# ndas7/Parallel-Systems-MPI-TFIDF

Hardware: AMD Instinct MI355X
Metric: corpus GB/s (TF-IDF hot path: tokenize->TF->DF->tf*idf->ordered output) (higher is better)
Workload: dtype u8/u32 (f64 score)

## Files before the change

parallel-systems-mpi-tfidf_amd/csrc/finalize.hip:

```cpp
#include "dev_common.h"
#include "dev_vocab.h"
#include "kernels.h"
#include "synth.h"

#include <type_traits>
#define G(p) ((GLOBAL_AS std::remove_pointer_t<decltype(p)>*)(p))
template <class T> __device__ __forceinline__ void sto(T* p, T v) { *(GLOBAL_AS T*)p = v; }

namespace {
constexpr int NT = 256;
inline unsigned grid_for(uint64_t n, int nt = NT) { return n ? (unsigned)((n + nt - 1) / nt) : 1u; }
inline int ok() { return hipGetLastError() == hipSuccess ? 0 : -1; }

__device__ __forceinline__ uint4 u128_from(uint64_t lo, uint64_t hi) {
    return make_uint4((uint32_t)lo, (uint32_t)(lo >> 32), (uint32_t)hi, (uint32_t)(hi >> 32));
}
__device__ __forceinline__ bool u128_eq(uint4 a, uint4 b) { return a.x == b.x && a.y == b.y && a.z == b.z && a.w == b.w; }
}


__global__ void k_vocab_flags(VocabDev v, uint64_t cap, uint32_t* __restrict__ flags) {
    uint64_t s = (uint64_t)blockIdx.x * blockDim.x + threadIdx.x;
    if (s >= cap) return;
    uint4 k = v.keys[s];
// ... 971 lines not shown
    k_df_mark<<<grid_for(V), NT, 0, s>>>(df, V, present);
    return ok();
}
__global__ void k_df_list(const uint32_t* __restrict__ ps, uint64_t nvals, uint32_t* __restrict__ vals) {
    const uint64_t stride = (uint64_t)gridDim.x * blockDim.x;
    for (uint64_t x = (uint64_t)blockIdx.x * blockDim.x + threadIdx.x; x < nvals; x += stride)
        if (ps[x + 1] != ps[x]) vals[ps[x]] = (uint32_t)x;
}
int launch_df_list(const uint32_t* present_scan, uint64_t nvals, uint32_t* vals, hipStream_t s) {
    const unsigned full = grid_for(nvals), cap = 1u << 20;
    k_df_list<<<full < cap ? full : cap, NT, 0, s>>>(present_scan, nvals, vals);
    return ok();
}


__global__ void k_doc_keys(const uint32_t* __restrict__ ids, uint32_t n, uint64_t* __restrict__ keys,
                           uint32_t* __restrict__ seq) {
    uint32_t i = blockIdx.x * blockDim.x + threadIdx.x;
    if (i >= n) return;
    uint32_t id = ids ? ids[i] : i + 1;
    uint32_t dg[10];
    int k = 0;
    do { dg[k++] = id % 10; id /= 10; } while (id);
    uint64_t key = 0;
    for (int p = 0; p < 10; ++p) key = key * 11 + (p < k ? dg[k - 1 - p] : 10u);
    keys[i] = key;
    seq[i] = i;
}
int launch_doc_keys(const uint32_t* doc_ids, uint32_t ndocs, uint64_t* keys, uint32_t* seq, hipStream_t s) {
    if (!ndocs) return 0;
    k_doc_keys<<<grid_for(ndocs), NT, 0, s>>>(doc_ids, ndocs, keys, seq);
    return ok();
}
__global__ void k_gather_meta(const uint32_t* __restrict__ order, const uint32_t* __restrict__ np,
                              const uint64_t* __restrict__ recoff, const uint32_t* __restrict__ dsize,
                              const uint8_t* __restrict__ flags, uint32_t n, uint64_t* __restrict__ out,
                              uint4* __restrict__ meta) {
    uint32_t i = blockIdx.x * blockDim.x + threadIdx.x;
    if (i >= n) return;
    const uint32_t d = order[i];
    const uint32_t c = np[d];
    const uint64_t rb = c ? recoff[d] : 0ull;
    out[i] = c;
    meta[i] = make_uint4((uint32_t)rb, (uint32_t)(rb >> 32), (c & 0x3FFFFFFFu) | ((uint32_t)(flags[d] & 3u) << 30), dsize[d]);
}
int launch_gather_meta(const uint32_t* order, const uint32_t* doc_npairs, const uint64_t* doc_recoff,
                       const uint32_t* doc_size, const uint8_t* doc_flags, uint32_t ndocs, uint64_t* npairs_ord,
                       uint4* meta, hipStream_t s) {
    if (!ndocs) return 0;
    k_gather_meta<<<grid_for(ndocs), NT, 0, s>>>(order, doc_npairs, doc_recoff, doc_size, doc_flags, ndocs,
                                                npairs_ord, meta);
    return ok();
}


constexpr int K5_MAX = K5_MAX_PAIRS;
constexpr uint32_t K5_SMALL = 64;
constexpr uint32_t K5_SMALL_DOC = 128;
constexpr uint32_t K5_PS_SPLIT = 4096;
constexpr uint32_t K5_WAVE = 1024;
constexpr uint32_t K5_IDX_BITS = 11;
constexpr int K5_BATCH = 8;
#ifndef K5_EB
#define K5_EB 4
#endif
#ifndef K5_EMIT
#define K5_EMIT 2
#endif
#ifndef K5_WPS
#define K5_WPS 4
#endif
#ifndef K5_WPS_WIDE
#define K5_WPS_WIDE 4
#endif
constexpr uint32_t K5_NB_BITS = 9;
constexpr uint32_t K5_NB = 1u << K5_NB_BITS;
constexpr uint32_t K5_GROUP_MAX = 48;
constexpr uint32_t K5L_GROUP_MAX = 32;
#ifndef K5L_EB
#define K5L_EB 8
#endif

__global__ void k_idf_of_rank(const uint32_t* __restrict__ df_of_rank, const uint32_t* __restrict__ idf_idx,
                              const double* __restrict__ idf, uint32_t V, double* __restrict__ out) {
    uint32_t r = blockIdx.x * blockDim.x + threadIdx.x;
    if (r < V) out[r] = idf_idx ? idf[idf_idx[df_of_rank[r]]] : idf[df_of_rank[r]];
}

template <bool BYDF>
__device__ __forceinline__ double k5_idf(const K5Args& a, uint32_t r) {
    if constexpr (BYDF) return G(a.idf)[G(a.df_of_rank)[r]];
    else return G(a.idf_rank)[r];
}

template <bool BYDF>
__device__ __forceinline__ void k5_emit(const K5Args& a, uint64_t o, double ds, uint32_t rank, uint32_t cnt) {
    const double tf = (double)cnt / ds;
    sto(&a.out_term[o], (uint32_t)(rank));
    sto(&a.out_cnt[o], (uint32_t)(cnt));
    sto(&a.out_score[o], (double)(tf * k5_idf<BYDF>(a, rank)));
}

__device__ __forceinline__ uint32_t k5_rank(const K5Args& a, uint32_t r) {
    if (r >= a.nterms) { atomicOr(a.status, ST_BOUNDS); r = 0; }
    return r;
}

constexpr uint32_t K5_WIDE_BITS = 32 - K5_IDX_BITS + K5_NB_BITS;
__device__ __forceinline__ bool k5_by_wave(const K5Args& a, uint32_t n, bool presorted) {
    if (presorted) return n <= K5_WAVE;
    return n <= K5_SMALL || (n <= K5_WAVE && a.rank_bits <= K5_WIDE_BITS);
}

__device__ __noinline__ void k5_radix(uint32_t rank_bits, const uint32_t* rec_cnt, const double* idf_rank,
                                      uint32_t* out_term, uint32_t* out_cnt, double* out_score, uint32_t* buf0,
                                      uint32_t* buf1, uint32_t* h, uint32_t n, uint64_t rb, uint64_t ob, double ds) {
    const uint32_t lane = threadIdx.x & 63;
    const uint64_t below = (1ull << lane) - 1ull;
    uint32_t cur = 0;
    for (uint32_t sh = K5_IDX_BITS; sh < K5_IDX_BITS + rank_bits; sh += 8) {
        const uint32_t* src = cur ? buf1 : buf0;
        uint32_t* dst = cur ? buf0 : buf1;
        h[4 * lane] = 0; h[4 * lane + 1] = 0; h[4 * lane + 2] = 0; h[4 * lane + 3] = 0;
        __builtin_amdgcn_fence(__ATOMIC_RELEASE, "wavefront");
        __builtin_amdgcn_fence(__ATOMIC_ACQUIRE, "wavefront");
        for (uint32_t j = lane; j < n; j += 64) atomicAdd(&h[(src[j] >> sh) & 0xFFu], 1u);
        __builtin_amdgcn_fence(__ATOMIC_RELEASE, "wavefront");
        __builtin_amdgcn_fence(__ATOMIC_ACQUIRE, "wavefront");
        {
            const uint32_t v0 = h[4 * lane], v1 = h[4 * lane + 1], v2 = h[4 * lane + 2], v3 = h[4 * lane + 3];
            const uint32_t tot = v0 + v1 + v2 + v3;
            const uint32_t ex = wave_incl_scan(tot) - tot;
            h[4 * lane] = ex; h[4 * lane + 1] = ex + v0; h[4 * lane + 2] = ex + v0 + v1; h[4 * lane + 3] = ex + v0 + v1 + v2;
        }
        __builtin_amdgcn_fence(__ATOMIC_RELEASE, "wavefront");
        __builtin_amdgcn_fence(__ATOMIC_ACQUIRE, "wavefront");
        for (uint32_t r0 = 0; r0 < n; r0 += 64) {
            const uint32_t j = r0 + lane;
            const bool valid = j < n;
            const uint32_t key = valid ? src[j] : 0u;
            const uint32_t dg = (key >> sh) & 0xFFu;
            uint64_t m = __ballot(valid);
#pragma unroll
            for (int b = 0; b < 8; ++b) {
                const bool bit = (dg >> b) & 1u;
                const uint64_t bb = __ballot(valid && bit);
                m &= bit ? bb : ~bb;
            }
            const uint32_t lrank = (uint32_t)__popcll(m & below);
            const uint32_t cnt = (uint32_t)__popcll(m);
            const uint32_t base = valid ? h[dg] : 0u;
            __builtin_amdgcn_fence(__ATOMIC_RELEASE, "wavefront");
            __builtin_amdgcn_fence(__ATOMIC_ACQUIRE, "wavefront");
            if (valid) {
                dst[base + lrank] = key;
                if (lrank == cnt - 1u) h[dg] = base + cnt;
            }
            __builtin_amdgcn_fence(__ATOMIC_RELEASE, "wavefront");
            __builtin_amdgcn_fence(__ATOMIC_ACQUIRE, "wavefront");
        }
        cur ^= 1u;
    }
    const uint32_t* fin = cur ? buf1 : buf0;
    for (uint32_t j0 = 0; j0 < n; j0 += 64 * K5_BATCH) {
        uint32_t key[K5_BATCH], cnt[K5_BATCH];
        double idf[K5_BATCH];
#pragma unroll
        for (int q = 0; q < K5_BATCH; ++q) {
// ... 698 lines not shown
            }
            __builtin_amdgcn_fence(__ATOMIC_RELEASE, "wavefront");
            __builtin_amdgcn_fence(__ATOMIC_ACQUIRE, "wavefront");
        }
#pragma unroll
        for (int q = 0; q < Q; ++q) {
            if (64u * q + lane < n) {
                const uint64_t o = D0.ob + pos[q];
                sto(&a.out_term[o], (uint32_t)(r0[q]));
                sto(&a.out_cnt[o], (uint32_t)(c0[q]));
                sto(&a.out_score[o], (double)(((double)c0[q] / D0.ds) * f0[q]));
            }
        }
        D0 = D1;
        D1 = D2;
#pragma unroll
        for (int q = 0; q < Q; ++q) {
            r0[q] = r1[q]; c0[q] = c1[q]; f0[q] = f1[q];
            r1[q] = r2[q]; c1[q] = c2[q];
        }
    }
}
template <bool BYDF>
__global__ __launch_bounds__(256) void k_emit_split(K5Args a) {
    const uint32_t nt = *a.split_count < a.split_cap ? *a.split_count : a.split_cap;
    for (uint32_t t = blockIdx.x; t < nt; t += gridDim.x) {
        const uint2 tk = a.split_tasks[t];
        const uint4 m = gload(a.meta + tk.x);
        const uint32_t n = m.z & 0x3FFFFFFFu;
        const uint64_t rb = ((uint64_t)m.y << 32) | m.x;
        const uint64_t ob = G(a.out_off)[tk.x];
        const double ds = (double)m.w;
        if (rb + n > a.rec_total) { if (threadIdx.x == 0) atomicOr(a.status, ST_BOUNDS); continue; }
        const uint32_t j1 = (tk.y + 1) * K5_PS_SPLIT < n ? (tk.y + 1) * K5_PS_SPLIT : n;
        for (uint32_t j0 = tk.y * K5_PS_SPLIT; j0 < j1; j0 += 256 * K5L_EB) {
            uint32_t rk[K5L_EB], cn[K5L_EB];
            double f[K5L_EB];
#pragma unroll
            for (int e = 0; e < K5L_EB; ++e) {
                const uint32_t j = j0 + 256u * e + threadIdx.x;
                rk[e] = j < j1 ? a.rec_slot[rb + j] : 0u;
                cn[e] = j < j1 ? a.rec_cnt[rb + j] : 0u;
            }
#pragma unroll
            for (int e = 0; e < K5L_EB; ++e) {
                const uint32_t j = j0 + 256u * e + threadIdx.x;
                if (j < j1) rk[e] = k5_rank(a, rk[e]);
                f[e] = j < j1 ? k5_idf<BYDF>(a, rk[e]) : 0.0;
            }
#pragma unroll
            for (int e = 0; e < K5L_EB; ++e) {
                const uint32_t j = j0 + 256u * e + threadIdx.x;
                if (j < j1) {
                    sto(&a.out_term[ob + j], (uint32_t)(rk[e]));
                    sto(&a.out_cnt[ob + j], (uint32_t)(cn[e]));
                    sto(&a.out_score[ob + j], (double)(((double)cn[e] / ds) * f[e]));
                }
            }
        }
    }
}
static void launch_score_wave(const K5Args& a, bool wide, uint32_t wg, hipStream_t s) {
    if (!wide) k_score_wave<false, false><<<wg, NT, 0, s>>>(a);
    else if (a.idf_by_df) k_score_wave<true, true><<<wg, NT, 0, s>>>(a);
    else k_score_wave<true, false><<<wg, NT, 0, s>>>(a);
}
static void launch_emit_split(const K5Args& a, int ncu, hipStream_t s) {
    if (a.idf_by_df) k_emit_split<true><<<(unsigned)ncu * 4u, 256, 0, s>>>(a);
    else k_emit_split<false><<<(unsigned)ncu * 4u, 256, 0, s>>>(a);
}
static void launch_score_large(const K5Args& a, uint32_t grid, hipStream_t s) {
    static_assert(K5_MAX % 2 == 0 && K5_MAX / 2 >= 1024, "k_score_large instances");
    if (a.idf_by_df) {
        k_score_large<(uint32_t)K5_MAX / 2, 10, true><<<grid, NT, 0, s>>>(a);
        k_score_large<(uint32_t)K5_MAX, 11, true><<<grid, NT, 0, s>>>(a);
    } else {
        k_score_large<(uint32_t)K5_MAX / 2, 10, false><<<grid, NT, 0, s>>>(a);
        k_score_large<(uint32_t)K5_MAX, 11, false><<<grid, NT, 0, s>>>(a);
    }
}
int launch_score_order(const K5Args& a, Arena& ar, hipStream_t s, hipStream_t s2, hipEvent_t ev_fork,
                       hipEvent_t ev_join) {
    if (!a.ndocs) return 0;
    {
        FillList fl{};
        fl.p[0] = a.large_count;
        fl.bytes[0] = 4;
        fl.n = 1;
        if (a.split_count) {
            fl.p[1] = a.split_count;
            fl.bytes[1] = 4;
            fl.n = 2;
        }
        if (launch_fill_multi(fl, s)) return -1;
    }
    if (!a.idf_by_df)
        k_idf_of_rank<<<grid_for(a.nterms ? a.nterms : 1), NT, 0, s>>>(a.df_of_rank, a.idf_idx, a.idf, a.nterms,
                                                                      a.idf_rank);
    static int ncu = 0;
    if (!ncu) {
        int dev = 0;
        if (hipGetDevice(&dev) != hipSuccess ||
            hipDeviceGetAttribute(&ncu, hipDeviceAttributeMultiprocessorCount, dev) != hipSuccess || ncu <= 0)
            ncu = 256;
    }
    const uint32_t wg_need = (a.ndocs + NT / 64 - 1) / (NT / 64);
    const bool wide = a.rank_bits + K5_IDX_BITS > 32;
    const uint32_t wg_cu = wide ? (uint32_t)K5_WPS_WIDE : 4u;
    const uint32_t wg = wg_need < (uint32_t)ncu * wg_cu ? wg_need : (uint32_t)ncu * wg_cu;
    const uint32_t grid = a.ndocs < 2048u ? a.ndocs : 2048u;
    K5Args hand = a;
    hand.cls_list = nullptr;
    if (!a.cls_list || !a.cls_off) return -1;
    k_k5_classify<<<a.cls_nblk, 256, 0, s>>>(a);
    if (scan_excl_u32(a.cls_off, a.cls_off, 3ull * a.cls_nblk + 1, ar, s)) return -1;
    k_k5_scatter<<<a.cls_nblk, 256, 0, s>>>(a);
    if (a.idf_by_df && !wide) return -1;
    if (a.idf_by_df) k_score_small<true><<<(unsigned)ncu * (unsigned)K5S_OCC, 256, 0, s>>>(a);
    else k_score_small<false><<<(unsigned)ncu * (unsigned)K5S_OCC, 256, 0, s>>>(a);
    launch_score_wave(a, wide, wg, s);
    if (a.split_count) launch_emit_split(a, ncu, s);
    launch_score_large(a, grid, s);
    if (wide) launch_score_large(hand, grid, s);
    return ok();
}


__global__ void k_keys_by_rank(const uint4* __restrict__ vkeys, const uint32_t* __restrict__ slot_of_rank, uint32_t V,
                               uint4* __restrict__ out) {
    uint32_t r = blockIdx.x * blockDim.x + threadIdx.x;
    if (r < V) out[r] = vkeys[slot_of_rank[r]];
}
int launch_keys_by_rank(const uint4* vkeys, const uint32_t* slot_of_rank, uint32_t V, uint4* out, hipStream_t s) {
    if (!V) return 0;
    k_keys_by_rank<<<grid_for(V), NT, 0, s>>>(vkeys, slot_of_rank, V, out);
    return ok();
}
__device__ __forceinline__ uint32_t owner_of(const uint4 k, uint32_t R) {
    const uint64_t lo = ((uint64_t)k.y << 32) | k.x, hi = ((uint64_t)k.w << 32) | k.z;
    const uint64_t h = mix64(lo ^ (hi * 0x9E3779B97F4A7C15ull) ^ 0x5851F42D4C957F2Dull);
    return (uint32_t)(((h >> 32) * (uint64_t)R) >> 32);
}
constexpr uint32_t XO_MAXR = 1024;
__device__ __forceinline__ uint4 owner_key(const OwnerKeySrc& ks, uint32_t i) {
    const uint4 s = gload(ks.skey + i);
    const uint32_t b15 = s.x & 0xFFu;
    if (b15 == 0x00u || b15 == 0x09u)
        return make_uint4(__builtin_bswap32(s.w), __builtin_bswap32(s.z), __builtin_bswap32(s.y), __builtin_bswap32(s.x));
    return gload(ks.vkeys + G(ks.slot_of_rank)[i]);
}
__global__ void k_owner_count(const OwnerKeySrc ks, uint32_t V, uint32_t R, uint32_t* __restrict__ cnt) {
    __shared__ uint32_t h[XO_MAXR];
    for (uint32_t o = threadIdx.x; o < R; o += blockDim.x) h[o] = 0;
    __syncthreads();
    for (uint32_t r = blockIdx.x * blockDim.x + threadIdx.x; r < V; r += gridDim.x * blockDim.x)
        atomicAdd(&h[owner_of(owner_key(ks, r), R)], 1u);
    __syncthreads();
    for (uint32_t o = threadIdx.x; o < R; o += blockDim.x)
        if (h[o]) atomicAdd(&cnt[o], h[o]);
}
__global__ void k_owner_scatter(const OwnerKeySrc ks, const uint32_t* __restrict__ df, uint32_t V, uint32_t R,
                                const uint32_t* __restrict__ cnt, uint32_t* __restrict__ cur, uint32_t* __restrict__ srec,
                                uint32_t* __restrict__ sidx) {
    __shared__ uint32_t h[XO_MAXR], base[XO_MAXR], seg[XO_MAXR];
    if (threadIdx.x == 0) {
        uint32_t acc = 0;
        for (uint32_t o = 0; o < R; ++o) { seg[o] = acc; acc += cnt[o]; }
    }
    for (uint32_t o = threadIdx.x; o < R; o += blockDim.x) h[o] = 0;
    __syncthreads();
    const uint32_t r0 = blockIdx.x * blockDim.x * 8;
    uint32_t own[8], pos[8];
#pragma unroll
    for (int q = 0; q < 8; ++q) {
        const uint32_t r = r0 + q * blockDim.x + threadIdx.x;
        own[q] = r < V ? owner_of(owner_key(ks, r), R) : 0xFFFFFFFFu;
        pos[q] = own[q] != 0xFFFFFFFFu ? atomicAdd(&h[own[q]], 1u) : 0u;
    }
    __syncthreads();
    for (uint32_t o = threadIdx.x; o < R; o += blockDim.x) base[o] = h[o] ? seg[o] + atomicAdd(&cur[o], h[o]) : 0u;
    __syncthreads();
// ... 695 lines not shown
```

parallel-systems-mpi-tfidf_amd/csrc/prims.hip:

```cpp
#include "prims.h"
#include "dev_common.h"

namespace {

constexpr int SC_NT = 256;
constexpr int SC_IT = 8;
constexpr int SC_TILE = SC_NT * SC_IT;

template <typename T>
__device__ __forceinline__ T wave_incl_scan_t(T v) {
    const int lane = threadIdx.x & 63;
#pragma unroll
    for (int o = 1; o < 64; o <<= 1) {
        T t = __shfl_up(v, o, 64);
        if (lane >= o) v += t;
    }
    return v;
}

template <typename T>
__device__ __forceinline__ T block_excl_scan_t(T v, T* wsum, T* total) {
    const int lane = threadIdx.x & 63, w = threadIdx.x >> 6;
    T inc = wave_incl_scan_t(v);
    if (lane == 63) wsum[w] = inc;
// ... 167 lines not shown
    for (int j = 0; j < RS_IT; ++j) {
        const uint64_t idx = wb + (uint64_t)j * 64 + lane;
        const bool valid = idx < n;
        k[j] = valid ? kin[idx] : K{};
        v[j] = valid ? vin[idx] : 0u;
        d[j] = valid ? digit_of(k[j], p) : 0u;
    }
#pragma unroll
    for (int j = 0; j < RS_IT; ++j) {
        const bool valid = wb + (uint64_t)j * 64 + lane < n;
        uint64_t m = __ballot(valid);
#pragma unroll
        for (int b = 0; b < 8; ++b) {
            const bool bit = (d[j] >> b) & 1u;
            const uint64_t bb = __ballot(valid && bit);
            m &= bit ? bb : ~bb;
        }
        const uint32_t lrank = (uint32_t)__popcll(m & lt);
        r[j] = valid ? wc[w][d[j]] + lrank : 0u;
        if (valid && lrank == 0) wc[w][d[j]] += (uint32_t)__popcll(m);
    }
    __syncthreads();
    {
        uint32_t c[RS_NT / 64], tot = 0;
#pragma unroll
        for (int q = 0; q < RS_NT / 64; ++q) { c[q] = wc[q][tid]; wc[q][tid] = tot; tot += c[q]; }
        uint32_t all;
        dstart[tid] = block_excl_scan<RS_NT>(tot, wsum, &all);
    }
    __syncthreads();
#pragma unroll
    for (int j = 0; j < RS_IT; ++j) {
        if (wb + (uint64_t)j * 64 + lane >= n) continue;
        const uint32_t pos = dstart[d[j]] + wc[w][d[j]] + r[j];
        sk[pos] = k[j];
        sv[pos] = v[j];
    }
    __syncthreads();
    const uint32_t tn = n - t0 < (uint64_t)RS_TILE ? (uint32_t)(n - t0) : (uint32_t)RS_TILE;
#pragma unroll
    for (int q = 0; q < RS_IT; ++q) {
        const uint32_t i = (uint32_t)tid + (uint32_t)q * RS_NT;
        if (i >= tn) continue;
        const K kk = sk[i];
        const uint32_t dd = digit_of(kk, p);
        const uint64_t o = (uint64_t)gbase[dd] + (i - dstart[dd]);
        kout[o] = kk;
        vout[o] = sv[i];
    }
}

template <typename K>
int radix_sort_t(K* k0, uint32_t* v0, K* k1, uint32_t* v1, uint64_t n, uint32_t byte_mask, int nbytes,
                 Arena& ar, hipStream_t s) {
    if (n <= 1 || byte_mask == 0) return 0;
    if (n > 0xFFFFFFFFull) return -3;
    uint32_t nb = (uint32_t)((n + RS_TILE - 1) / RS_TILE);
    size_t m = ar.mark();
    uint32_t* hist = (uint32_t*)ar.get(((uint64_t)256 * nb + 1) * sizeof(uint32_t));
    if (!hist) return -2;
    int cur = 0;
    for (int p = 0; p < nbytes; ++p) {
        if (!((byte_mask >> p) & 1u)) continue;
        K* ki = cur ? k1 : k0;
        uint32_t* vi = cur ? v1 : v0;
        K* ko = cur ? k0 : k1;
        uint32_t* vo = cur ? v0 : v1;
        k_rs_hist<K><<<nb, RS_NT, 0, s>>>(ki, n, p, hist, nb);
        if (nb <= RS_FUSED_MAXNB) {
            k_rs_scatter<K, true><<<nb, RS_NT, 0, s>>>(ki, vi, ko, vo, n, p, hist, nb);
        } else {
            int rc = scan_excl_t<uint32_t>(hist, hist, (uint64_t)256 * nb, ar, s);
            if (rc) return rc;
            k_rs_scatter<K, false><<<nb, RS_NT, 0, s>>>(ki, vi, ko, vo, n, p, hist, nb);
        }
        cur ^= 1;
    }
    ar.release(m);
    return hipGetLastError() == hipSuccess ? cur : -1;
}

constexpr int TS_NT = 1024;
constexpr uint32_t TS_T = 2048;

__device__ __forceinline__ bool key_lt(uint64_t a, uint64_t b) { return a < b; }
__device__ __forceinline__ bool key_eq(uint64_t a, uint64_t b) { return a == b; }
__device__ __forceinline__ bool key_lt(uint4 a, uint4 b) {
    if (a.w != b.w) return a.w < b.w;
    if (a.z != b.z) return a.z < b.z;
    if (a.y != b.y) return a.y < b.y;
    return a.x < b.x;
}
__device__ __forceinline__ bool key_eq(uint4 a, uint4 b) { return a.x == b.x && a.y == b.y && a.z == b.z && a.w == b.w; }
__device__ __forceinline__ void key_max(uint64_t& k) { k = ~0ull; }
__device__ __forceinline__ void key_max(uint4& k) { k = make_uint4(~0u, ~0u, ~0u, ~0u); }

template <typename K>
__global__ __launch_bounds__(TS_NT) void k_tile_sort(const K* __restrict__ kin, const uint32_t* __restrict__ vin,
                                                    uint64_t n, K* __restrict__ tk, uint32_t* __restrict__ tv,
                                                    uint32_t* __restrict__ ti) {
    __shared__ K sk[TS_T];
    __shared__ uint32_t sv[TS_T], si[TS_T];
    const uint32_t tid = threadIdx.x;
    const uint64_t t0 = (uint64_t)blockIdx.x * TS_T;
#pragma unroll
    for (uint32_t h = 0; h < 2; ++h) {
        const uint32_t e = tid + h * TS_NT;
        const uint64_t g = t0 + e;
        if (g < n) { sk[e] = kin[g]; sv[e] = vin[g]; si[e] = (uint32_t)g; }
        else { K m; key_max(m); sk[e] = m; sv[e] = 0u; si[e] = 0xFFFFFFFFu; }
    }
    __syncthreads();
    for (uint32_t k = 2; k <= TS_T; k <<= 1) {
        for (uint32_t j = k >> 1; j > 0; j >>= 1) {
            const uint32_t i = 2u * tid - (tid & (j - 1u)), l = i + j;
            const bool asc = (i & k) == 0u;
            const K a = sk[i], b = sk[l];
            const uint32_t ia = si[i], ib = si[l];
            const bool b_first = key_lt(b, a) || (key_eq(a, b) && ib < ia);
            if (b_first == asc) {
                sk[i] = b; sk[l] = a;
                si[i] = ib; si[l] = ia;
                const uint32_t x = sv[i]; sv[i] = sv[l]; sv[l] = x;
            }
            __syncthreads();
        }
    }
#pragma unroll
    for (uint32_t h = 0; h < 2; ++h) {
        const uint32_t e = tid + h * TS_NT;
        const uint64_t g = t0 + e;
        if (g < n) { tk[g] = sk[e]; tv[g] = sv[e]; ti[g] = si[e]; }
    }
}

constexpr uint32_t TS_LB = 8;
template <typename K>
__global__ __launch_bounds__(256) void k_tile_rank(const K* __restrict__ tk, const uint32_t* __restrict__ ti,
                                                  uint64_t n, uint32_t* __restrict__ pos) {
    const uint64_t g = (uint64_t)blockIdx.x * blockDim.x + threadIdx.x;
    if (g >= n) return;
    const uint32_t t = (uint32_t)(g / TS_T), nt = (uint32_t)((n + TS_T - 1) / TS_T);
    const uint32_t b0 = blockIdx.y * TS_LB;
    const K key = tk[g];
    const uint32_t idx = ti[g];
    uint32_t lo[TS_LB], len[TS_LB];
#pragma unroll
    for (uint32_t q = 0; q < TS_LB; ++q) {
        const uint32_t b = b0 + q;
        const uint64_t st = (uint64_t)b * TS_T;
        lo[q] = 0;
        len[q] = (b < nt && b != t) ? (uint32_t)((n - st) < TS_T ? (n - st) : TS_T) : 0u;
    }
    for (uint32_t it = 0; it < 12; ++it) {
#pragma unroll
        for (uint32_t q = 0; q < TS_LB; ++q) {
            if (len[q] == 0u) continue;
            const uint32_t half = len[q] >> 1, mid = lo[q] + half;
            const uint64_t e = (uint64_t)(b0 + q) * TS_T + mid;
            const K m = tk[e];
            const bool before = key_lt(m, key) || (key_eq(m, key) && ti[e] < idx);
            if (before) { lo[q] = mid + 1u; len[q] -= half + 1u; }
            else len[q] = half;
        }
    }
    uint32_t c = blockIdx.y == 0 ? (uint32_t)(g - (uint64_t)t * TS_T) : 0u;
#pragma unroll
    for (uint32_t q = 0; q < TS_LB; ++q) c += lo[q];
    if (c) atomicAdd(&pos[g], c);
}
template <typename K>
__global__ void k_tile_place(const K* __restrict__ tk, const uint32_t* __restrict__ tv,
                             const uint32_t* __restrict__ pos, uint64_t n, K* __restrict__ kout,
                             uint32_t* __restrict__ vout) {
    const uint64_t g = (uint64_t)blockIdx.x * blockDim.x + threadIdx.x;
    if (g >= n) return;
    const uint32_t p = pos[g];
    kout[p] = tk[g];
    vout[p] = tv[g];
}

template <typename K>
int tile_sort_t(const K* k0, const uint32_t* v0, K* k1, uint32_t* v1, uint64_t n, Arena& ar, hipStream_t s) {
    if (n == 0) return 1;
    const uint32_t nt = (uint32_t)((n + TS_T - 1) / TS_T);
    size_t m = ar.mark();
    K* tk = (K*)ar.get(n * sizeof(K));
    uint32_t* tv = (uint32_t*)ar.get(n * 4);
    uint32_t* ti = (uint32_t*)ar.get(n * 4);
    if (!tk || !tv || !ti) return -2;
    uint32_t* pos = (uint32_t*)ar.get(n * 4);
    if (!pos) return -2;
    if (hipMemsetAsync(pos, 0, n * 4, s) != hipSuccess) return -1;
    k_tile_sort<K><<<nt, TS_NT, 0, s>>>(k0, v0, n, tk, tv, ti);
    k_tile_rank<K><<<dim3((unsigned)((n + 255) / 256), (nt + TS_LB - 1) / TS_LB), 256, 0, s>>>(tk, ti, n, pos);
    k_tile_place<K><<<(unsigned)((n + 255) / 256), 256, 0, s>>>(tk, tv, pos, n, k1, v1);
    ar.release(m);
    return hipGetLastError() == hipSuccess ? 1 : -1;
}

__global__ __launch_bounds__(256) void k_orand_u64(const uint64_t* __restrict__ k, uint64_t n, unsigned long long* acc) {
    __shared__ unsigned long long sa[4], so[4];
    uint64_t a = ~0ull, o = 0;
    for (uint64_t i = (uint64_t)blockIdx.x * blockDim.x + threadIdx.x; i < n; i += (uint64_t)gridDim.x * blockDim.x) {
        a &= k[i];
        o |= k[i];
    }
    for (int off = 32; off > 0; off >>= 1) {
        a &= __shfl_xor(a, off, 64);
        o |= __shfl_xor(o, off, 64);
    }
    const int w = threadIdx.x >> 6;
    if ((threadIdx.x & 63) == 0) { sa[w] = a; so[w] = o; }
    __syncthreads();
    if (threadIdx.x == 0) {
        atomicAnd(&acc[0], sa[0] & sa[1] & sa[2] & sa[3]);
        atomicOr(&acc[1], so[0] | so[1] | so[2] | so[3]);
    }
}

__global__ __launch_bounds__(256) void k_orand_u128(const uint4* __restrict__ k, uint64_t n, unsigned long long* acc) {
    __shared__ unsigned long long s4[4][4];
    uint64_t a0 = ~0ull, a1 = ~0ull, o0 = 0, o1 = 0;
    for (uint64_t i = (uint64_t)blockIdx.x * blockDim.x + threadIdx.x; i < n; i += (uint64_t)gridDim.x * blockDim.x) {
        uint4 v = k[i];
        uint64_t lo = ((uint64_t)v.y << 32) | v.x, hi = ((uint64_t)v.w << 32) | v.z;
        a0 &= lo; a1 &= hi; o0 |= lo; o1 |= hi;
    }
    for (int off = 32; off > 0; off >>= 1) {
        a0 &= __shfl_xor(a0, off, 64); a1 &= __shfl_xor(a1, off, 64);
        o0 |= __shfl_xor(o0, off, 64); o1 |= __shfl_xor(o1, off, 64);
    }
    const int w = threadIdx.x >> 6;
    if ((threadIdx.x & 63) == 0) { s4[w][0] = a0; s4[w][1] = a1; s4[w][2] = o0; s4[w][3] = o1; }
    __syncthreads();
    if (threadIdx.x == 0) {
        atomicAnd(&acc[0], s4[0][0] & s4[1][0] & s4[2][0] & s4[3][0]);
        atomicAnd(&acc[1], s4[0][1] & s4[1][1] & s4[2][1] & s4[3][1]);
        atomicOr(&acc[2], s4[0][2] | s4[1][2] | s4[2][2] | s4[3][2]);
        atomicOr(&acc[3], s4[0][3] | s4[1][3] | s4[2][3] | s4[3][3]);
    }
}

}

int scan_excl_u32(const uint32_t* in, uint32_t* out, uint64_t n, Arena& ar, hipStream_t s) {
    return scan_excl_t<uint32_t>(in, out, n, ar, s);
}
int scan_excl_u64(const uint64_t* in, uint64_t* out, uint64_t n, Arena& ar, hipStream_t s) {
    return scan_excl_t<uint64_t>(in, out, n, ar, s);
}
int tile_sort_u64(const uint64_t* k0, const uint32_t* v0, uint64_t* k1, uint32_t* v1, uint64_t n, Arena& ar,
                  hipStream_t s) {
    if (n > SORT_TILE_MAXN) return -3;
    if (n <= 1) {
        if (n == 1 && (hipMemcpyAsync(k1, k0, 8, hipMemcpyDeviceToDevice, s) != hipSuccess ||
                       hipMemcpyAsync(v1, v0, 4, hipMemcpyDeviceToDevice, s) != hipSuccess)) return -1;
        return 1;
    }
    return tile_sort_t<uint64_t>(k0, v0, k1, v1, n, ar, s);
}
int tile_sort_u128(const uint4* k0, const uint32_t* v0, uint4* k1, uint32_t* v1, uint64_t n, Arena& ar,
                   hipStream_t s) {
    if (n > SORT_TILE_MAXN) return -3;
    if (n <= 1) {
        if (n == 1 && (hipMemcpyAsync(k1, k0, 16, hipMemcpyDeviceToDevice, s) != hipSuccess ||
                       hipMemcpyAsync(v1, v0, 4, hipMemcpyDeviceToDevice, s) != hipSuccess)) return -1;
        return 1;
    }
    return tile_sort_t<uint4>(k0, v0, k1, v1, n, ar, s);
}
int radix_sort_u64(uint64_t* k0, uint32_t* v0, uint64_t* k1, uint32_t* v1, uint64_t n, uint32_t byte_mask,
                   Arena& ar, hipStream_t s) {
    return radix_sort_t<uint64_t>(k0, v0, k1, v1, n, byte_mask, 8, ar, s);
}
int radix_sort_u128(uint4* k0, uint32_t* v0, uint4* k1, uint32_t* v1, uint64_t n, uint32_t byte_mask,
                    Arena& ar, hipStream_t s) {
    return radix_sort_t<uint4>(k0, v0, k1, v1, n, byte_mask, 16, ar, s);
}
// ... 75 lines not shown
```

Before: 337.2.

## Fuse tile-sort rank and place into block-level merge-path kernel, drop value shuffling

Replaces the per-element global binary-search ranking kernel plus separate placement kernel with one kernel. In it, each 256-key block finds its window in every other tile using wave-cooperative 64-way search, then ranks window elements against the block's keys held in LDS, and scatters directly. The tile sort stops carrying values through the bitonic network, gathers them by original index instead, and uses wavefront barriers for small strides. A single-tile fast path skips the rank pass entirely. Separately, zeroing of the counters is folded into the idf kernel to save a fill launch. The cost is a much more intricate kernel with LDS sizing tied to SORT_TILE_MAXN, plus a fallback path for wide windows.

```diff
diff --git a/parallel-systems-mpi-tfidf_amd/csrc/finalize.hip b/parallel-systems-mpi-tfidf_amd/csrc/finalize.hip
--- a/parallel-systems-mpi-tfidf_amd/csrc/finalize.hip
+++ b/parallel-systems-mpi-tfidf_amd/csrc/finalize.hip
@@ -1077,8 +1077,13 @@
 #endif
 
 __global__ void k_idf_of_rank(const uint32_t* __restrict__ df_of_rank, const uint32_t* __restrict__ idf_idx,
-                              const double* __restrict__ idf, uint32_t V, double* __restrict__ out) {
+                              const double* __restrict__ idf, uint32_t V, double* __restrict__ out,
+                              uint32_t* __restrict__ z0, uint32_t* __restrict__ z1) {
     uint32_t r = blockIdx.x * blockDim.x + threadIdx.x;
+    if (r == 0) {
+        *z0 = 0u;
+        if (z1) *z1 = 0u;
+    }
     if (r < V) out[r] = idf_idx ? idf[idf_idx[df_of_rank[r]]] : idf[df_of_rank[r]];
 }
 
@@ -1943,7 +1948,10 @@
 int launch_score_order(const K5Args& a, Arena& ar, hipStream_t s, hipStream_t s2, hipEvent_t ev_fork,
                        hipEvent_t ev_join) {
     if (!a.ndocs) return 0;
-    {
+    if (!a.idf_by_df) {
+        k_idf_of_rank<<<grid_for(a.nterms ? a.nterms : 1), NT, 0, s>>>(a.df_of_rank, a.idf_idx, a.idf, a.nterms,
+                                                                      a.idf_rank, a.large_count, a.split_count);
+    } else {
         FillList fl{};
         fl.p[0] = a.large_count;
         fl.bytes[0] = 4;
@@ -1955,9 +1963,6 @@
         }
         if (launch_fill_multi(fl, s)) return -1;
     }
-    if (!a.idf_by_df)
-        k_idf_of_rank<<<grid_for(a.nterms ? a.nterms : 1), NT, 0, s>>>(a.df_of_rank, a.idf_idx, a.idf, a.nterms,
-                                                                      a.idf_rank);
     static int ncu = 0;
     if (!ncu) {
         int dev = 0;
diff --git a/parallel-systems-mpi-tfidf_amd/csrc/prims.hip b/parallel-systems-mpi-tfidf_amd/csrc/prims.hip
--- a/parallel-systems-mpi-tfidf_amd/csrc/prims.hip
+++ b/parallel-systems-mpi-tfidf_amd/csrc/prims.hip
@@ -273,119 +273,265 @@
 
 constexpr int TS_NT = 1024;
 constexpr uint32_t TS_T = 2048;
-
-__device__ __forceinline__ bool key_lt(uint64_t a, uint64_t b) { return a < b; }
-__device__ __forceinline__ bool key_eq(uint64_t a, uint64_t b) { return a == b; }
-__device__ __forceinline__ bool key_lt(uint4 a, uint4 b) {
-    if (a.w != b.w) return a.w < b.w;
-    if (a.z != b.z) return a.z < b.z;
-    if (a.y != b.y) return a.y < b.y;
-    return a.x < b.x;
-}
-__device__ __forceinline__ bool key_eq(uint4 a, uint4 b) { return a.x == b.x && a.y == b.y && a.z == b.z && a.w == b.w; }
+constexpr uint32_t TS_WSPAN = 128;
+
 __device__ __forceinline__ void key_max(uint64_t& k) { k = ~0ull; }
 __device__ __forceinline__ void key_max(uint4& k) { k = make_uint4(~0u, ~0u, ~0u, ~0u); }
+__device__ __forceinline__ uint64_t key_hi(uint64_t k) { return k; }
+__device__ __forceinline__ uint64_t key_hi(uint4 k) { return ((uint64_t)k.w << 32) | k.z; }
+__device__ __forceinline__ bool pair_before(uint64_t a, uint32_t ia, uint64_t b, uint32_t ib) {
+    return (a < b) | ((a == b) & (ia < ib));
+}
+__device__ __forceinline__ bool pair_before(uint4 a, uint32_t ia, uint4 b, uint32_t ib) {
+    const uint64_t ah = ((uint64_t)a.w << 32) | a.z, al = ((uint64_t)a.y << 32) | a.x;
+    const uint64_t bh = ((uint64_t)b.w << 32) | b.z, bl = ((uint64_t)b.y << 32) | b.x;
+    return (ah < bh) | ((ah == bh) & ((al < bl) | ((al == bl) & (ia < ib))));
+}
 
 template <typename K>
 __global__ __launch_bounds__(TS_NT) void k_tile_sort(const K* __restrict__ kin, const uint32_t* __restrict__ vin,
-                                                    uint64_t n, K* __restrict__ tk, uint32_t* __restrict__ tv,
-                                                    uint32_t* __restrict__ ti) {
+                                                    uint64_t n, uint32_t tl, K* __restrict__ tk,
+                                                    uint32_t* __restrict__ ti, uint32_t* __restrict__ vout) {
     __shared__ K sk[TS_T];
-    __shared__ uint32_t sv[TS_T], si[TS_T];
+    __shared__ uint32_t si[TS_T];
     const uint32_t tid = threadIdx.x;
-    const uint64_t t0 = (uint64_t)blockIdx.x * TS_T;
+    const uint64_t t0 = (uint64_t)blockIdx.x * tl;
 #pragma unroll
     for (uint32_t h = 0; h < 2; ++h) {
         const uint32_t e = tid + h * TS_NT;
         const uint64_t g = t0 + e;
-        if (g < n) { sk[e] = kin[g]; sv[e] = vin[g]; si[e] = (uint32_t)g; }
-        else { K m; key_max(m); sk[e] = m; sv[e] = 0u; si[e] = 0xFFFFFFFFu; }
-    }
-    __syncthreads();
+        if (e < tl && g < n) { sk[e] = kin[g]; si[e] = (uint32_t)g; }
+        else { K m; key_max(m); sk[e] = m; si[e] = 0xFFFFFFFFu; }
+    }
+    lds_barrier();
     for (uint32_t k = 2; k <= TS_T; k <<= 1) {
         for (uint32_t j = k >> 1; j > 0; j >>= 1) {
             const uint32_t i = 2u * tid - (tid & (j - 1u)), l = i + j;
             const bool asc = (i & k) == 0u;
             const K a = sk[i], b = sk[l];
             const uint32_t ia = si[i], ib = si[l];
-            const bool b_first = key_lt(b, a) || (key_eq(a, b) && ib < ia);
-            if (b_first == asc) {
+            if (pair_before(b, ib, a, ia) == asc) {
                 sk[i] = b; sk[l] = a;
                 si[i] = ib; si[l] = ia;
-                const uint32_t x = sv[i]; sv[i] = sv[l]; sv[l] = x;
-            }
-            __syncthreads();
+            }
+            const uint32_t nj = j > 1u ? j >> 1 : k;
+            if (j >= TS_WSPAN || nj >= TS_WSPAN) lds_barrier();
+            else {
+                __builtin_amdgcn_fence(__ATOMIC_RELEASE, "wavefront");
+                __builtin_amdgcn_wave_barrier();
+                __builtin_amdgcn_fence(__ATOMIC_ACQUIRE, "wavefront");
+            }
         }
     }
 #pragma unroll
     for (uint32_t h = 0; h < 2; ++h) {
         const uint32_t e = tid + h * TS_NT;
         const uint64_t g = t0 + e;
-        if (g < n) { tk[g] = sk[e]; tv[g] = sv[e]; ti[g] = si[e]; }
-    }
-}
-
-constexpr uint32_t TS_LB = 8;
+        if (e >= tl || g >= n) continue;
+        const uint32_t src = si[e];
+        tk[g] = sk[e];
+        if (vout) vout[g] = src < n ? vin[src] : 0u;
+        else ti[g] = src;
+    }
+}
+
+constexpr int TR_NT = 1024;
+constexpr uint32_t TR_K = 256;
+constexpr uint32_t TR_U = 8;
+constexpr uint32_t TR_SR = 2u * 64u / (TR_NT / 64u);
+constexpr uint32_t TR_WMAX = 512;
+constexpr uint32_t TR_FL = 4;
+constexpr uint32_t TR_MAXT = (uint32_t)(SORT_TILE_MAXN / TS_T);
 template <typename K>
-__global__ __launch_bounds__(256) void k_tile_rank(const K* __restrict__ tk, const uint32_t* __restrict__ ti,
-                                                  uint64_t n, uint32_t* __restrict__ pos) {
-    const uint64_t g = (uint64_t)blockIdx.x * blockDim.x + threadIdx.x;
-    if (g >= n) return;
-    const uint32_t t = (uint32_t)(g / TS_T), nt = (uint32_t)((n + TS_T - 1) / TS_T);
-    const uint32_t b0 = blockIdx.y * TS_LB;
-    const K key = tk[g];
-    const uint32_t idx = ti[g];
-    uint32_t lo[TS_LB], len[TS_LB];
-#pragma unroll
-    for (uint32_t q = 0; q < TS_LB; ++q) {
-        const uint32_t b = b0 + q;
-        const uint64_t st = (uint64_t)b * TS_T;
-        lo[q] = 0;
-        len[q] = (b < nt && b != t) ? (uint32_t)((n - st) < TS_T ? (n - st) : TS_T) : 0u;
-    }
-    for (uint32_t it = 0; it < 12; ++it) {
-#pragma unroll
-        for (uint32_t q = 0; q < TS_LB; ++q) {
-            if (len[q] == 0u) continue;
-            const uint32_t half = len[q] >> 1, mid = lo[q] + half;
-            const uint64_t e = (uint64_t)(b0 + q) * TS_T + mid;
-            const K m = tk[e];
-            const bool before = key_lt(m, key) || (key_eq(m, key) && ti[e] < idx);
-            if (before) { lo[q] = mid + 1u; len[q] -= half + 1u; }
-            else len[q] = half;
-        }
-    }
-    uint32_t c = blockIdx.y == 0 ? (uint32_t)(g - (uint64_t)t * TS_T) : 0u;
-#pragma unroll
-    for (uint32_t q = 0; q < TS_LB; ++q) c += lo[q];
-    if (c) atomicAdd(&pos[g], c);
-}
-template <typename K>
-__global__ void k_tile_place(const K* __restrict__ tk, const uint32_t* __restrict__ tv,
-                             const uint32_t* __restrict__ pos, uint64_t n, K* __restrict__ kout,
-                             uint32_t* __restrict__ vout) {
-    const uint64_t g = (uint64_t)blockIdx.x * blockDim.x + threadIdx.x;
-    if (g >= n) return;
-    const uint32_t p = pos[g];
-    kout[p] = tk[g];
-    vout[p] = tv[g];
+__global__ __launch_bounds__(TR_NT) void k_tile_rank_place(const K* __restrict__ tk, const uint32_t* __restrict__ ti,
+                                                          const uint32_t* __restrict__ vin, uint64_t n, uint32_t tl,
+                                                          K* __restrict__ kout, uint32_t* __restrict__ vout) {
+    __shared__ K bk[TR_K];
+    __shared__ uint64_t bh[TR_K];
+    __shared__ uint32_t bi[TR_K];
+    __shared__ uint32_t wlo[TR_MAXT], whi[TR_MAXT], woff[TR_MAXT + 1], big[TR_MAXT];
+    __shared__ uint32_t hist[TR_K + 1], fwd[TR_K];
+    __shared__ uint32_t wsum[TR_NT / 64];
+    __shared__ uint32_t sbase, nbig;
+    const uint32_t tid = threadIdx.x, lane = tid & 63u;
+    const uint32_t t = blockIdx.y, nt = gridDim.y, kb0 = blockIdx.x * TR_K;
+    const uint64_t ts = (uint64_t)t * tl;
+    const uint32_t tn = n - ts < (uint64_t)tl ? (uint32_t)(n - ts) : tl;
+    if (kb0 >= tn) return;
+    const uint32_t nk = tn - kb0 < TR_K ? tn - kb0 : TR_K;
+    const uint64_t g = ts + kb0 + tid;
+    K key;
+    key_max(key);
+    uint32_t idx = 0xFFFFFFFFu;
+    if (tid < TR_K) {
+        if (tid < nk) { key = tk[g]; idx = ti[g]; }
+        bk[tid] = key;
+        bh[tid] = key_hi(key);
+        bi[tid] = idx;
+        hist[tid] = 0;
+        fwd[tid] = 0;
+    }
+    if (tid == 0) hist[TR_K] = 0;
+    if (tid < TR_MAXT) { wlo[tid] = 0; whi[tid] = 0; }
+    lds_barrier();
+    uint32_t val = 0;
+    if (tid < nk && idx < n) val = vin[idx];
+    {
+        const uint32_t wv = tid >> 6;
+        uint32_t lo[TR_SR], hi[TR_SR];
+#pragma unroll
+        for (uint32_t r = 0; r < TR_SR; ++r) {
+            const uint32_t sid = wv + r * (TR_NT / 64u), b = sid >> 1;
+            const uint64_t st = (uint64_t)b * tl;
+            lo[r] = 0;
+            hi[r] = (b < nt && b != t) ? (uint32_t)(n - st < (uint64_t)tl ? n - st : (uint64_t)tl) : 0u;
+        }
+        for (;;) {
+            uint32_t rem = 0;
+#pragma unroll
+            for (uint32_t r = 0; r < TR_SR; ++r) rem |= hi[r] - lo[r];
+            if (!__any(rem != 0u)) break;
+            K pk[TR_SR];
+            uint32_t pi[TR_SR];
+#pragma unroll
+            for (uint32_t r = 0; r < TR_SR; ++r) {
+                const uint32_t b = (wv + r * (TR_NT / 64u)) >> 1;
+                const uint32_t len = hi[r] - lo[r];
+                const uint64_t e = len ? (uint64_t)b * tl + lo[r] + len * (lane + 1u) / 65u : 0u;
+                pk[r] = tk[e];
+                pi[r] = ti[e];
+            }
+#pragma unroll
+            for (uint32_t r = 0; r < TR_SR; ++r) {
+                const uint32_t w = (wv + r * (TR_NT / 64u)) & 1u;
+                const uint32_t len = hi[r] - lo[r];
+                const bool pred = len && pair_before(pk[r], pi[r], bk[w ? nk - 1u : 0u], bi[w ? nk - 1u : 0u]);
+                const uint32_t c = (uint32_t)__popcll(__ballot(pred));
+                if (len) {
+                    const uint32_t nlo = c ? lo[r] + len * c / 65u + 1u : lo[r];
+                    hi[r] = c < 64u ? lo[r] + len * (c + 1u) / 65u : hi[r];
+                    lo[r] = nlo;
+                }
+            }
+        }
+#pragma unroll
+        for (uint32_t r = 0; r < TR_SR; ++r) {
+            const uint32_t sid = wv + r * (TR_NT / 64u), b = sid >> 1, w = sid & 1u;
+            if (lane == 0 && b < nt && b != t) { if (w) whi[b] = lo[r]; else wlo[b] = lo[r]; }
+        }
+    }
+    lds_barrier();
+    if (tid < 64u) {
+        const uint32_t l = wlo[tid], u = whi[tid];
+        const uint32_t wd = u > l ? u - l : 0u;
+        const bool wide = wd > TR_WMAX;
+        const uint32_t inc = wave_incl_scan(wide ? 0u : wd);
+        woff[tid + 1u] = inc;
+        if (tid == 0) woff[0] = 0;
+        const uint32_t sl = wave_sum(l);
+        const uint64_t bal = __ballot(wide);
+        if (wide) big[__popcll(bal & ((1ull << tid) - 1ull))] = tid;
+        if (tid == 0) { sbase = sl; nbig = (uint32_t)__popcll(bal); }
+    }
+    lds_barrier();
+    const uint32_t S = woff[TR_MAXT];
+    for (uint32_t e0 = 0; e0 < S; e0 += TR_NT * TR_U) {
+        K x[TR_U];
+        uint64_t xh[TR_U];
+        uint32_t xi[TR_U], lo[TR_U], len[TR_U];
+#pragma unroll
+        for (uint32_t u = 0; u < TR_U; ++u) {
+            const uint32_t e = e0 + u * TR_NT + tid;
+            lo[u] = 0;
+            len[u] = e < S ? nk : 0u;
+            xi[u] = 0;
+            key_max(x[u]);
+            if (e < S) {
+                uint32_t b = 0;
+#pragma unroll
+                for (uint32_t stp = TR_MAXT / 2; stp; stp >>= 1)
+                    if (woff[b + stp] <= e) b += stp;
+                const uint64_t ge = (uint64_t)b * tl + wlo[b] + (e - woff[b]);
+                x[u] = tk[ge];
+                xi[u] = ti[ge];
+            }
+            xh[u] = key_hi(x[u]);
+        }
+        for (uint32_t it = 0; it < 9; ++it) {
+#pragma unroll
+            for (uint32_t u = 0; u < TR_U; ++u) {
+                if (len[u] == 0u) continue;
+                const uint32_t half = len[u] >> 1, mid = lo[u] + half;
+                const uint64_t h = bh[mid];
+                bool before = h < xh[u];
+                if (h == xh[u]) before = pair_before(bk[mid], bi[mid], x[u], xi[u]);
+                if (before) { lo[u] = mid + 1u; len[u] -= half + 1u; }
+                else len[u] = half;
+            }
+        }
+#pragma unroll
+        for (uint32_t u = 0; u < TR_U; ++u)
+            if (e0 + u * TR_NT + tid < S) atomicAdd(&hist[lo[u]], 1u);
+    }
+    const uint32_t nb = nbig;
+    if (nb) {
+        constexpr uint32_t NQ = TR_NT / TR_K;
+        const uint32_t i = tid % TR_K;
+        const K x = bk[i];
+        const uint32_t xi = bi[i];
+        uint32_t sum = 0;
+        for (uint32_t j0 = tid / TR_K; j0 < nb; j0 += NQ * TR_FL) {
+            uint64_t st[TR_FL];
+            uint32_t lo[TR_FL], len[TR_FL];
+#pragma unroll
+            for (uint32_t q = 0; q < TR_FL; ++q) {
+                const uint32_t j = j0 + q * NQ;
+                const bool on = j < nb && i < nk;
+                const uint32_t b = big[j < nb ? j : 0u];
+                st[q] = (uint64_t)b * tl + wlo[b];
+                lo[q] = 0;
+                len[q] = on ? whi[b] - wlo[b] : 0u;
+            }
+            for (uint32_t it = 0; it < 12; ++it) {
+#pragma unroll
+                for (uint32_t q = 0; q < TR_FL; ++q) {
+                    if (len[q] == 0u) continue;
+                    const uint32_t half = len[q] >> 1, mid = lo[q] + half;
+                    const uint64_t e = st[q] + mid;
+                    if (pair_before(tk[e], ti[e], x, xi)) { lo[q] = mid + 1u; len[q] -= half + 1u; }
+                    else len[q] = half;
+                }
+            }
+#pragma unroll
+            for (uint32_t q = 0; q < TR_FL; ++q) sum += lo[q];
+        }
+        if (sum) atomicAdd(&fwd[i], sum);
+    }
+    lds_barrier();
+    const uint32_t h = tid < TR_K ? hist[tid] : 0u;
+    uint32_t tot;
+    const uint32_t before = block_excl_scan<TR_NT, true>(h, wsum, &tot) + h;
+    if (tid < nk) {
+        const uint64_t p = (uint64_t)(kb0 + tid) + sbase + before + fwd[tid];
+        if (p < n && idx < n) { kout[p] = key; vout[p] = val; }
+    }
 }
 
 template <typename K>
 int tile_sort_t(const K* k0, const uint32_t* v0, K* k1, uint32_t* v1, uint64_t n, Arena& ar, hipStream_t s) {
     if (n == 0) return 1;
     const uint32_t nt = (uint32_t)((n + TS_T - 1) / TS_T);
+    const uint32_t tl = (uint32_t)((n + nt - 1) / nt);
+    if (nt == 1) {
+        k_tile_sort<K><<<1, TS_NT, 0, s>>>(k0, v0, n, tl, k1, nullptr, v1);
+        return hipGetLastError() == hipSuccess ? 1 : -1;
+    }
     size_t m = ar.mark();
     K* tk = (K*)ar.get(n * sizeof(K));
-    uint32_t* tv = (uint32_t*)ar.get(n * 4);
     uint32_t* ti = (uint32_t*)ar.get(n * 4);
-    if (!tk || !tv || !ti) return -2;
-    uint32_t* pos = (uint32_t*)ar.get(n * 4);
-    if (!pos) return -2;
-    if (hipMemsetAsync(pos, 0, n * 4, s) != hipSuccess) return -1;
-    k_tile_sort<K><<<nt, TS_NT, 0, s>>>(k0, v0, n, tk, tv, ti);
-    k_tile_rank<K><<<dim3((unsigned)((n + 255) / 256), (nt + TS_LB - 1) / TS_LB), 256, 0, s>>>(tk, ti, n, pos);
-    k_tile_place<K><<<(unsigned)((n + 255) / 256), 256, 0, s>>>(tk, tv, pos, n, k1, v1);
+    if (!tk || !ti) return -2;
+    k_tile_sort<K><<<nt, TS_NT, 0, s>>>(k0, v0, n, tl, tk, ti, nullptr);
+    k_tile_rank_place<K><<<dim3((tl + TR_K - 1) / TR_K, nt), TR_NT, 0, s>>>(tk, ti, v0, n, tl, k1, v1);
     ar.release(m);
     return hipGetLastError() == hipSuccess ? 1 : -1;
 }
```

Result: faster. 340.9, median of 6 (+1.1%).
